# ferdean/lsa-fw

Hardware: AMD Instinct MI355X
Metric: converged eigenpairs/sec (k=20, shift-invert) (higher is better)
Workload: dtype c128

## Files before the change

lsa-fw_amd/csrc/dense.hip:

```cpp
#include <algorithm>
#include <chrono>
#include <cmath>
#include <cstdint>
#include <cstring>
#include <vector>

#include "lsa_internal.h"

namespace {

struct Z {
    double re, im;
};
inline Z operator+(Z a, Z b) { return {a.re + b.re, a.im + b.im}; }
inline Z operator-(Z a, Z b) { return {a.re - b.re, a.im - b.im}; }
inline Z operator-(Z a) { return {-a.re, -a.im}; }
inline Z operator*(Z a, Z b) { return {a.re * b.re - a.im * b.im, a.re * b.im + a.im * b.re}; }
inline Z operator*(double a, Z b) { return {a * b.re, a * b.im}; }
inline Z conj(Z a) { return {a.re, -a.im}; }
inline double abs1(Z a) { return std::fabs(a.re) + std::fabs(a.im); }
inline double abs2(Z a) { return a.re * a.re + a.im * a.im; }
inline double zabs(Z a) { return std::hypot(a.re, a.im); }
inline Z zdiv(Z a, Z b) {
    if (std::fabs(b.re) >= std::fabs(b.im)) {
// ... 921 lines not shown
    double* est_out;
    lsa_ks_result* result;
    int32_t m = 0;
    int64_t n = 0;
    int nev = 0, ldh = 0;
    double keep_fraction = 0.5;
    Selector sel;
    Rng rng;
    std::vector<Z> vec, H, T, Q, S, b, bq, w;
    std::vector<double> est, rel, keys;
    std::vector<int> rank;
    std::vector<char> select;
    int kept = 0, restarts = 0;
    int64_t applies = 0;
    KsClock clk;

    void random_vector() {
        for (int64_t i = 0; i < n; ++i) {
            rng.normal_pair(vec[(size_t)i].re, vec[(size_t)i].im);
            if (mask && mask[i] == 0.0) vec[(size_t)i] = {0.0, 0.0};
        }
    }
    int init(const char* who, const void* v0) {
        LSA_CHECK(lsa_krylov_shape(k, &n, &m));
        if (m > n) return lsa_set_error(ctx, LSA_ERR_ARG, "ncv = %d exceeds the problem size %lld", m, (long long)n);
        LSA_CHECK(ks_check_options(ctx, who, o, max_out, theta_out, lambda_out));
        nev = std::min<int>(o->nev, m);
        keep_fraction = ks_keep_fraction(o);
        sel = Selector{o->which, o->transform, {o->sigma[0], o->sigma[1]}, {o->antishift[0], o->antishift[1]}, {o->target[0], o->target[1]}};
        rng = ks_rng(o);
// ... 16 lines not shown
        select.resize((size_t)m);
        memset(result, 0, sizeof *result);
        return LSA_OK;
    }
    int extend(int j, int32_t* bd) {
        LSA_CHECK(lsa_krylov_extend(ctx, k, j, m, H.data(), ldh, bd));
        if (*bd >= 0) H[(size_t)*bd * ldh + (size_t)*bd + 1] = {0.0, 0.0};
        return (int)LSA_OK;
    }
    int inject_random(int j) {
        random_vector();
        return lsa_krylov_inject(ctx, k, j, vec.data());
    }
    int expand() {
        clk.start();
        LSA_CHECK(ks_expand(kept, m, &applies, [&](int j, int32_t* bd) { return extend(j, bd); }, [&](int j) { return inject_random(j); }));
        clk.lap(clk.expand);
        return LSA_OK;
    }
    int expand_after(int rc0, int32_t bd0, double seconds, int64_t* later_steps) {
        bool first = true;
        const int64_t before = applies + (bd0 < 0 ? m - kept : bd0 - kept + 1);
        *later_steps = 0;
        clk.start();
        LSA_CHECK(ks_expand(kept, m, &applies,
                            [&](int j, int32_t* bd) {
                                if (!first) return extend(j, bd);
                                first = false;
                                LSA_CHECK(rc0);
                                *bd = bd0;
// ... 2 lines not shown
                            },
                            [&](int j) { return inject_random(j); }));
        clk.lap(clk.expand);
        clk.expand += seconds;
        *later_steps = applies - before;
        return LSA_OK;
    }
    int after_expand(const char* who, bool* done) {
        const Mat Hm{H.data(), ldh}, Tm{T.data(), m}, Qm{Q.data(), m}, Sm{S.data(), m};
        *done = false;
        clk.start();
        for (int c = 0; c < m; ++c) {
            b[(size_t)c] = Hm(m, c);
            for (int r = 0; r < m; ++r) Tm(r, c) = Hm(r, c);
        }
        if (!schur(m, Tm, Qm)) return lsa_set_error(ctx, LSA_ERR_DIVERGED, "Krylov-Schur: the QR algorithm on the projected matrix did not converge");
        tri_eigenvectors(m, Tm, Sm);
        for (int c = 0; c < m; ++c) {
            Z acc = {0.0, 0.0};
            for (int r = 0; r < m; ++r) acc = acc + b[(size_t)r] * Qm(r, c);
            bq[(size_t)c] = acc;
        }
        for (int c = 0; c < m; ++c) {
            Z acc = {0.0, 0.0};
            for (int r = 0; r <= c; ++r) acc = acc + bq[(size_t)r] * Sm(r, c);
            est[(size_t)c] = zabs(acc);
            w[(size_t)c] = Tm(c, c);
            keys[(size_t)c] = sel.key(w[(size_t)c]);
            rel[(size_t)c] = est[(size_t)c] / std::max(zabs(w[(size_t)c]), 2.2250738585072014e-308);
        }
// ... 20 lines not shown
            clk.lap(clk.dense);
            ks_fill_result(result, clk, nconv, nout, restarts, applies, nconv < m ? rel[(size_t)rank[(size_t)nconv]] : 0.0);
            *done = true;
            return k_agree_in_step(ctx, who);
        }
        int knew = ks_keep_count(m, nconv, keep_fraction);
        {
            std::vector<double> sorted(keys);
            std::sort(sorted.begin(), sorted.end());
            const double thr = sorted[(size_t)knew] > sorted[(size_t)knew - 1] ? 0.5 * (sorted[(size_t)knew - 1] + sorted[(size_t)knew]) : sorted[(size_t)knew - 1];
            for (int c = 0; c < m; ++c) select[(size_t)c] = keys[(size_t)c] <= thr;
            const int sdim = schur_reorder(m, Tm, Qm, select);
            knew = std::max(std::min(sdim, m - 1), 1);
        }
        clk.lap(clk.dense);
        LSA_CHECK(lsa_krylov_restart(ctx, k, m, knew, Q.data(), m));
        clk.lap(clk.restart);
        std::fill(H.begin(), H.end(), Z{0.0, 0.0});
        for (int c = 0; c < knew; ++c) {
            for (int r = 0; r <= c; ++r) Hm(r, c) = Tm(r, c);
            Z acc = {0.0, 0.0};
            for (int r = 0; r < m; ++r) acc = acc + b[(size_t)r] * Qm(r, c);
            Hm(knew, c) = acc;
        }
        kept = knew;
        ++restarts;
        return LSA_OK;
    }
};

}

extern "C" {

int lsa_krylov_solve(lsa_ctx* ctx, lsa_krylov* k, const lsa_ks_options* o, const void* v0, const double* mask, int32_t max_out, void* theta_out,
                     void* lambda_out, void* X_out, double* est_out, lsa_ks_result* result) {
    if (!ctx || !k || !o || !result) return lsa_set_error(ctx, LSA_ERR_ARG, "lsa_krylov_solve: null argument");
    KsState st{ctx, k, o, mask, max_out, theta_out, lambda_out, X_out, est_out, result};
    LSA_CHECK(st.init("lsa_krylov_solve", v0));
    for (bool done = false; !done;) {
        LSA_CHECK(st.expand());
        LSA_CHECK(st.after_expand("lsa_krylov_solve", &done));
    }
    return LSA_OK;
}

static_assert(sizeof(lsa_ks_batch_info) == 288, "lsa_ks_batch_info layout is part of the C-ABI (tests/test_lockstep_cpu.py)");
static_assert(sizeof(((lsa_ks_batch_info*)nullptr)->lockstep_steps) == 8 * kKrylovGroupMax && sizeof(((lsa_ks_batch_info*)nullptr)->solo_steps) == 8 * kKrylovGroupMax,
              "the per-problem counters of lsa_ks_batch_info hold one entry per problem of a group");

int lsa_krylov_solve_batch(lsa_ctx* ctx, int32_t J, lsa_krylov* const* k, const lsa_ks_options* const* opts, const void* const* v0, int32_t max_out,
                           void* const* theta_out, void* const* lambda_out, void* const* X_out, double* const* est_out, lsa_ks_result* results,
                           int32_t* status, lsa_ks_batch_info* info) {
    if (!ctx || !k || !opts || !results || !status) return lsa_set_error(ctx, LSA_ERR_ARG, "lsa_krylov_solve_batch: null argument");
    if (J < 1 || J > kKrylovGroupMax) return lsa_set_error(ctx, LSA_ERR_ARG, "lsa_krylov_solve_batch: J = %d outside [1, %d]", J, kKrylovGroupMax);
    if (max_out > 0 && (!theta_out || !lambda_out)) return lsa_set_error(ctx, LSA_ERR_ARG, "lsa_krylov_solve_batch: output buffers are required");
    for (int32_t z = 0; z < J; ++z)
        if (!opts[z]) return lsa_set_error(ctx, LSA_ERR_ARG, "lsa_krylov_solve_batch: null options (problem %d)", z);
    LSA_CHECK(krylov_group_check(ctx, J, k));
// ... 152 lines not shown
```

lsa-fw_amd/csrc/lsa_internal.h:

```cpp
#pragma once

#include <hip/hip_runtime.h>

#include <cstdarg>
#include <cstdint>
#include <cstdio>
#include <cstdlib>
#include <cstring>
#include <memory>
#include <string>
#include <vector>

#include "../../include/lsa_hip.h"

struct cplx {
    double re, im;
};
static_assert(sizeof(cplx) == 16, "complex128 layout");

__host__ __device__ inline cplx make_cplx(double r, double i) { return cplx{r, i}; }

template <typename T>
struct scalar_traits;
template <>
// ... 214 lines not shown
int k_dcgs2_tail_batch(lsa_ctx* ctx, int J, int64_t n, const int32_t* j, void* const* V, int64_t ldv, const void* const* y, void* const* work,
                       const lsa_mat* const* M, const lsa_mat* const* C, void* const* t, double* const* tail_part, void* const* slot, int lds);
int k_spmv_plain_subwave_lanes(const lsa_mat* A);
int k_basis_gemm_max_cols(int dtype);
int k_basis_gemm(lsa_ctx* ctx, int dtype, int64_t n, int m, int k, const void* V, int64_t ldv, const void* Q, int ldq,
                 void* Out, int64_t ldo);
int k_scatter_rows(lsa_ctx* ctx, int dtype, int64_t n, int ncols, const int32_t* perm, const void* In, void* Out);

int basis_upload_row_permutation(lsa_ctx* ctx, const char* who, int64_t n, const int32_t* perm, int32_t** row_perm);
int basis_times_host_matrix(lsa_ctx* ctx, int dtype, int64_t n, int m, int k, const void* V, const void* Q, int ldq, void* qdev, void* Out,
                            size_t pinned_extra);
int direct_solve_enqueue(lsa_ctx* ctx, lsa_op* op, int dtype, const void* rhs, void* y, void* z, void* r, bool refine, double* norms,
                         int direction = -1);
void stats_book_direct_solve(lsa_stats* st, int products, bool refine, double res, double bnorm);

struct KrylovGroupBuf {
    int32_t J, slots, nparts;
    void* Hdev;
    double *checks, *tail_parts;
};
int krylov_group_check(lsa_ctx* ctx, int32_t J, lsa_krylov* const* ks);
int krylov_group_alloc(lsa_ctx* ctx, int32_t J, lsa_krylov* const* ks, KrylovGroupBuf* gb);
void krylov_group_free(KrylovGroupBuf* gb);
int krylov_extend_batch(lsa_ctx* ctx, KrylovGroupBuf* gb, lsa_krylov* const* ks, const uint8_t* active, const int32_t* j0, int32_t j1, void* const* Hs,
                        int32_t ldh, int32_t* breakdown, int32_t* status, std::string* errs, lsa_ks_batch_info* info);
void lsa_name_problem(lsa_ctx* ctx, int32_t z);

struct lsa_ndlu;
struct lsa_op_parts {
    int64_t n;
// ... 74 lines not shown
```

lsa-fw_amd/csrc/solver.hip:

```cpp
#include <algorithm>
#include <chrono>
#include <cmath>
#include <complex>

#include "lsa_internal.h"

int ilu_check_abort(lsa_ctx* ctx, lsa_ilu* pc);
bool nd_batch_compatible(const lsa_ndlu* f, const lsa_ndlu* g);
int ndlu_solve_batch_dev(lsa_ctx* ctx, int32_t J, lsa_ndlu* const* f, int vdtype, const void** b, void* const* x);
int k_allgather_inplace(lsa_ctx* ctx, void* vec, size_t bytes_per_rank);

namespace {

using zc = std::complex<double>;
inline size_t esize(int dtype) { return dtype == LSA_C128 ? 16 : 8; }
inline double now_s() {
    return std::chrono::duration<double>(std::chrono::steady_clock::now().time_since_epoch()).count();
}

struct KrylovSwitches {
    bool fused;
    bool four_passes;
    bool tail;
    bool delayed;
    bool timing;
};
const KrylovSwitches& krylov_switches() {
    static const KrylovSwitches sw = [] {
        const char* passes = getenv("LSA_KRYLOV_PASSES");
        return KrylovSwitches{env_flag("LSA_KRYLOV_FUSED", true), passes && atoi(passes) == 4, env_flag("LSA_KRYLOV_TAIL", true),
                              env_flag("LSA_KRYLOV_DELAYED", true), getenv("LSA_KRYLOV_TIMING") != nullptr};
    }();
    return sw;
}

struct OrthWork {
    void *h1 = nullptr, *h2 = nullptr, *hcol = nullptr;
    double* nrm2 = nullptr;
    void* fused = nullptr;
    int cap = 0;
    int ensure_fused(lsa_ctx* ctx, int64_t n) {
        if (fused) return LSA_OK;
        LSA_HIP_ALLOC(ctx, hipMalloc(&fused, k_cgs2_fused_work_bytes(ctx, n, cap)));
        return LSA_OK;
    }
    int alloc(lsa_ctx* ctx, int cap_, int dtype) {
// ... 404 lines not shown
    int32_t* row_perm = nullptr;
    void *V, *V2, *w, *qdev;
    OrthWork ow;
    std::vector<zc> hcol;
    double* imag2 = nullptr;
    void* xtmp = nullptr;
    std::vector<double> imag_norms;
    void* Hdev = nullptr;
    double* checks = nullptr;
    int32_t batch = 0;
    bool pipeline = false;
    void* w2 = nullptr;
    double* tail_parts = nullptr;
    int32_t tail_nparts = 0;
    int32_t t_for = -1;
};

static size_t krylov_slot_bytes(int32_t ncv) { return (size_t)(2 * ncv + 4) * 16; }

static void krylov_free(lsa_krylov* k) {
    for (void* p : {k->V, k->V2, k->w, k->qdev, k->Hdev, (void*)k->checks, (void*)k->imag2, k->xtmp, (void*)k->row_perm, k->w2, (void*)k->tail_parts})
        if (p) (void)hipFree(p);
    k->ow.release();
    delete k;
}

extern "C" {

int lsa_gmres(lsa_ctx* ctx, const lsa_mat* C, lsa_ilu* pc, const lsa_vec* b, lsa_vec* x, int use_x0, double rtol, int restart,
              int maxit, int32_t* iters, double* rel_res) {
    if (!ctx || !C || !b || !x) return lsa_set_error(ctx, LSA_ERR_ARG, "lsa_gmres: null argument");
    if (C->n != C->ncols || b->n != C->n || x->n != C->n || b->dtype != x->dtype)
        return lsa_set_error(ctx, LSA_ERR_ARG, "lsa_gmres: shape/dtype mismatch");
    if (C->dtype == LSA_C128 && b->dtype != LSA_C128) return lsa_set_error(ctx, LSA_ERR_ARG, "lsa_gmres: complex matrix needs complex vectors");
    if (restart < 1 || maxit < 1 || !(rtol > 0.0)) return lsa_set_error(ctx, LSA_ERR_ARG, "lsa_gmres: restart, maxit, rtol must be positive");
    restart = std::min(restart, maxit);
    if (restart > k_basis_gemm_max_cols(b->dtype))
// ... 367 lines not shown
    return LSA_OK;
}

int lsa_krylov_create(lsa_ctx* ctx, lsa_op* op, int32_t ncv, lsa_krylov** out) {
    if (!ctx || !op || !out || ncv < 1) return lsa_set_error(ctx, LSA_ERR_ARG, "lsa_krylov_create: bad argument");
    if (ncv > k_basis_gemm_max_cols(LSA_C128))
        return lsa_set_error(ctx, LSA_ERR_ARG, "lsa_krylov_create: ncv=%d, the basis product handles at most %d basis vectors", ncv, k_basis_gemm_max_cols(LSA_C128));
    const size_t vb = (size_t)std::max<int64_t>(op->n, 1) * 16;
    const char* be = getenv("LSA_KRYLOV_BATCH");
    const int32_t batch = be && *be ? std::max(0, std::min(atoi(be), 256)) : 16;
    if (lsa_krylov* c = ctx->krylov_cache) {
        ctx->krylov_cache = nullptr;
        if (c->n == op->n && c->ncv == ncv && c->batch == batch) {
            c->op = op;
            c->pipeline = true;
            c->imag_norms.clear();
            (void)hipMemsetAsync(c->w, 0, vb, ctx->stream);
            *out = c;
            return LSA_OK;
        }
        krylov_free(c);
    }
    lsa_krylov* k = new lsa_krylov();
    k->ctx = ctx;
    k->op = op;
    k->n = op->n;
    k->ncv = ncv;
    k->V = k->V2 = k->w = k->qdev = nullptr;
    bool ok = hipMalloc(&k->V, vb * (size_t)(ncv + 1)) == hipSuccess && hipMalloc(&k->V2, vb * (size_t)(ncv + 1)) == hipSuccess &&
              hipMalloc(&k->w, vb) == hipSuccess && hipMalloc(&k->qdev, (size_t)(ncv + 1) * (size_t)(ncv + 1) * 16) == hipSuccess;
    if (!ok || k->ow.alloc(ctx, ncv + 1, LSA_C128) != LSA_OK) {
        lsa_krylov_destroy(k);
        return lsa_set_error(ctx, LSA_ERR_HIP, "lsa_krylov_create: out of device memory (n=%lld, ncv=%d)", (long long)op->n, ncv);
    }
    (void)hipMemsetAsync(k->w, 0, vb, ctx->stream);
    k->hcol.assign((size_t)ncv + 2, zc(0));
    k->batch = batch;
    const size_t slots = (size_t)std::max(batch, 1);
    if (hipMalloc(&k->Hdev, slots * krylov_slot_bytes(ncv)) != hipSuccess || hipMalloc((void**)&k->checks, slots * 2 * sizeof(double)) != hipSuccess) {
        lsa_krylov_destroy(k);
        return lsa_set_error(ctx, LSA_ERR_HIP, "lsa_krylov_create: out of device memory (pipeline buffers)");
    }
    k->pipeline = true;
    *out = k;
    return LSA_OK;
}

void lsa_krylov_destroy(lsa_krylov* k) {
    if (!k) return;
    lsa_ctx* ctx = k->ctx;
    if (ctx && ctx->stream) (void)hipStreamSynchronize(ctx->stream);
    if (k->row_perm) (void)hipFree(k->row_perm);
    k->row_perm = nullptr;
// ... 15 lines not shown

int lsa_krylov_shape(const lsa_krylov* k, int64_t* n, int32_t* ncv) {
    if (!k) return LSA_ERR_ARG;
    if (n) *n = k->n;
    if (ncv) *ncv = k->ncv;
    return LSA_OK;
}

int lsa_krylov_set_row_permutation(lsa_ctx* ctx, lsa_krylov* k, const int32_t* perm) {
    if (!ctx || !k) return lsa_set_error(ctx, LSA_ERR_ARG, "lsa_krylov_set_row_permutation: null argument");
    return basis_upload_row_permutation(ctx, "lsa_krylov_set_row_permutation", k->n, perm, &k->row_perm);
}

int lsa_krylov_set_start(lsa_ctx* ctx, lsa_krylov* k, const void* host_v) {
    if (!ctx || !k || !host_v) return lsa_set_error(ctx, LSA_ERR_ARG, "lsa_krylov_set_start: null argument");
    LSA_HIP_CHECK(ctx, hipMemcpyAsync(k->w, host_v, (size_t)k->n * 16, hipMemcpyHostToDevice, ctx->stream));
    double nrm = 0.0;
    LSA_CHECK(device_norm(ctx, LSA_C128, k->n, k->w, k->ow.nrm2, &nrm));
    if (!(nrm > 0.0) || !std::isfinite(nrm)) return lsa_set_error(ctx, LSA_ERR_ARG, "lsa_krylov_set_start: start vector is zero or not finite");
    LSA_CHECK(k_scale_by_inv_norm(ctx, LSA_C128, k->n, k->w, k->ow.nrm2, k->V));
    LSA_HIP_CHECK(ctx, hipStreamSynchronize(ctx->stream));
    k->pipeline = true;
    return LSA_OK;
}

int lsa_krylov_inject(lsa_ctx* ctx, lsa_krylov* k, int32_t j, const void* host_v) {
    if (!ctx || !k || !host_v) return lsa_set_error(ctx, LSA_ERR_ARG, "lsa_krylov_inject: null argument");
    if (j < 0 || j > k->ncv) return lsa_set_error(ctx, LSA_ERR_ARG, "lsa_krylov_inject: index %d out of range", j);
    if (j == 0) return lsa_krylov_set_start(ctx, k, host_v);
    const size_t vb = (size_t)k->n * 16;
    LSA_HIP_CHECK(ctx, hipMemcpyAsync(k->w, host_v, vb, hipMemcpyHostToDevice, ctx->stream));
    LSA_CHECK(orthonormalize(ctx, LSA_C128, k->n, k->V, k->n, j, k->w, (char*)k->V + (size_t)j * vb, k->ow, k->hcol.data()));
    const double beta = k->hcol[j].real();
    if (!(beta > 0.0) || !std::isfinite(beta)) return lsa_set_error(ctx, LSA_ERR_ARG, "lsa_krylov_inject: vector lies in the span of the basis");
    return LSA_OK;
}

enum class Orth {
    cgs2_fused,
    cgs2_staged,
    dcgs2,
};
struct StepPlan {
    bool pipelined = false;
// ... 12 lines not shown
    p.tail = p.pipelined && sw.tail && sw.fused && op->Kmul && !op->adjoint && !op->keep && !op->refine && op->n == k->n &&
             k_cgs2_tail_fits(ctx, k->n, k->ncv, op->Kmul, op->Kfac);
    return p;
}

static int krylov_enqueue_step(lsa_ctx* ctx, lsa_krylov* k, const StepPlan& plan, int32_t j, int32_t slot, bool first) {
    lsa_op* op = k->op;
    const int dtype = LSA_C128;
    const size_t vb = (size_t)k->n * 16;
    const void* vj = (char*)k->V + (size_t)j * vb;
    void* vn = (char*)k->V + (size_t)(j + 1) * vb;
    void* sl = (char*)k->Hdev + (size_t)slot * krylov_slot_bytes(k->ncv);
    double* chk = k->checks + 2 * (size_t)slot;
    const bool dcgs2 = plan.orth == Orth::dcgs2;
    if (plan.orth != Orth::cgs2_staged) LSA_CHECK(k->ow.ensure_fused(ctx, k->n));
    if (plan.tail) {
        if (k->t_for != j) LSA_CHECK(spmv_global(ctx, op->Kmul, dtype, vj, op->t, false));
        k->t_for = -1;
        LSA_CHECK(pc_global(ctx, pc_of(op), op->Kfac->row0, op->n, dtype, op->t, k->w));
        double* parts = k->tail_parts + (size_t)slot * 2 * (size_t)k->tail_nparts;
        if (dcgs2) {
            LSA_CHECK(k_dcgs2_step(ctx, k->n, j, k->V, k->n, k->w, first ? 1 : 0, sl, k->ncv, k->ow.fused, nullptr, nullptr, nullptr));
            LSA_CHECK(k_dcgs2_tail(ctx, k->n, j, k->V, k->n, k->w, k->ow.fused, op->Kmul, op->Kfac, op->t, parts, sl, k->ncv));
        } else {
            LSA_CHECK(k_cgs2_fused_tail(ctx, k->n, j + 1, k->V, k->n, k->w, k->w2, vn, sl, k->ow.fused, op->Kmul, op->Kfac, op->t, parts));
        }
        k->t_for = j + 1;
        return LSA_OK;
    }
    k->t_for = -1;
    const void* rhs = vj;
    if (op->Kmul) {
        LSA_CHECK(spmv_global(ctx, op->Kmul, dtype, vj, op->t, op->adjoint));
        rhs = op->t;
// ... 60 lines not shown

static int arnoldi_nonfinite(lsa_ctx* ctx, int32_t j) { return lsa_set_error(ctx, LSA_ERR_NONFINITE, "Arnoldi: non-finite norm at step %d", j); }

struct ExtendCursor {
    int32_t j;
    bool pending;
};

static int pipelined_prepare(lsa_ctx* ctx, lsa_krylov* k, const StepPlan& plan) {
    lsa_op* op = k->op;
    if (!op->gw_ready) {
        LSA_CHECK(op->gw.alloc(ctx, op->n, std::max(1, std::min({op->opts.ksp_restart, op->opts.ksp_maxit, 40})), LSA_C128));
        op->gw_ready = true;
    }
    if (plan.tail && !k->tail_parts) {
        const int32_t slots = std::max(k->batch, 1);
        k->tail_nparts = k_cgs2_tail_parts(k->n);
        LSA_HIP_ALLOC(ctx, hipMalloc(&k->w2, (size_t)k->n * 16));
        LSA_HIP_ALLOC(ctx, hipMalloc((void**)&k->tail_parts, (size_t)slots * 2 * (size_t)k->tail_nparts * sizeof(double)));
    }
    return LSA_OK;
}

static int accept_steps(lsa_ctx* ctx, lsa_krylov* k, const HessView& H, bool delayed, const char* slots, size_t slot_stride, const double* chk,
                        size_t chk_stride, int32_t nb, ExtendCursor* c, int32_t* breakdown, int32_t* accepted_out) {
    lsa_op* op = k->op;
    const double rtol = op->opts.ksp_rtol;
    cplx* hwork = (cplx*)k->hcol.data();
    const int32_t j = c->j;
    int32_t accepted = 0;
    *accepted_out = 0;
    for (int32_t s = 0; s < nb; ++s, ++accepted) {
        const cplx* hc = (const cplx*)(slots + (size_t)s * slot_stride);
        const bool first = s == 0 && !c->pending;
        if (delayed && !first) {
// ... 19 lines not shown
            *breakdown = j + s;
            return LSA_OK;
        }
    }
    c->j = j + accepted;
    *accepted_out = accepted;
    if (accepted < nb) k->t_for = -1;
    return LSA_OK;
}

static int extend_pipelined(lsa_ctx* ctx, lsa_krylov* k, const HessView& H, ExtendCursor* c, int32_t j1, int32_t* breakdown) {
    StepPlan plan = step_plan(ctx, k);
    LSA_CHECK(pipelined_prepare(ctx, k, plan));
    const int32_t slots = std::max(k->batch, 1);
    const size_t colb = krylov_slot_bytes(k->ncv);
    LSA_CHECK(lsa_ensure_scratch(ctx, 0, (size_t)slots * (colb + 2 * sizeof(double))));
    const bool delayed = plan.orth == Orth::dcgs2;
    char* host = (char*)ctx->pinned;
    k->t_for = -1;
    for (; c->j < j1 && plan.pipelined; plan = step_plan(ctx, k)) {
        const int32_t nb = std::min<int32_t>(slots, j1 - c->j);
        const double tq = now_s();
        for (int32_t s = 0; s < nb; ++s) {
            const int rc = krylov_enqueue_step(ctx, k, plan, c->j + s, s, s == 0 && !c->pending);
            if (rc != LSA_OK) {
                (void)hipStreamSynchronize(ctx->stream);
                return rc;
            }
        }
        if (plan.tail) LSA_CHECK(k_cgs2_tail_checks(ctx, nb, k->tail_nparts, k->tail_parts, k->checks));
        LSA_HIP_CHECK(ctx, hipMemcpyAsync(host, k->Hdev, (size_t)nb * colb, hipMemcpyDeviceToHost, ctx->stream));
        LSA_HIP_CHECK(ctx, hipMemcpyAsync(host + (size_t)slots * colb, k->checks, (size_t)nb * 2 * sizeof(double), hipMemcpyDeviceToHost, ctx->stream));
        const double tw = now_s();
        LSA_HIP_CHECK(ctx, hipStreamSynchronize(ctx->stream));
        if (krylov_switches().timing) fprintf(stderr, "[lsa_krylov] %d steps queued in %.3f ms, waited %.3f ms\n", nb, 1e3 * (tw - tq), 1e3 * (now_s() - tw));
        int32_t accepted = 0;
        LSA_CHECK(accept_steps(ctx, k, H, delayed, host, colb, (const double*)(host + (size_t)slots * colb), 2, nb, c, breakdown, &accepted));
        if (*breakdown >= 0) return LSA_OK;
    }
    if (c->pending) {
        const int32_t j = c->j;
        LSA_CHECK(k_dcgs2_step(ctx, k->n, j, k->V, k->n, nullptr, 0, k->Hdev, k->ncv, k->ow.fused, nullptr, nullptr, nullptr));
        LSA_HIP_CHECK(ctx, hipMemcpyAsync(host, k->Hdev, colb, hipMemcpyDeviceToHost, ctx->stream));
        LSA_HIP_CHECK(ctx, hipStreamSynchronize(ctx->stream));
        c->pending = false;
        const int what = finish_column(H, j, (const cplx*)host);
        if (what < 0) return arnoldi_nonfinite(ctx, j - 1);
        if (what > 0) *breakdown = j - 1;
    }
    return LSA_OK;
}

static int extend_one_step(lsa_ctx* ctx, lsa_krylov* k, const HessView& H, int32_t j, int32_t j1, int32_t* breakdown) {
    const size_t vb = (size_t)k->n * 16;
    k->t_for = -1;
    for (; j < j1; ++j) {
        const void* vj = (char*)k->V + (size_t)j * vb;
        void* vn = (char*)k->V + (size_t)(j + 1) * vb;
        LSA_CHECK(op_apply_dev(ctx, k->op, vj, k->w));
        LSA_CHECK(orthonormalize(ctx, LSA_C128, k->n, k->V, k->n, j + 1, k->w, vn, k->ow, k->hcol.data()));
        const int what = take_column(H, j, (const cplx*)k->hcol.data());
        if (what < 0) return arnoldi_nonfinite(ctx, j);
        if (what > 0) {
            *breakdown = j;
            break;
        }
    }
    return LSA_OK;
}

static int extend_rest(lsa_ctx* ctx, lsa_krylov* k, const HessView& H, ExtendCursor* c, int32_t j1, int32_t* bd) {
    int rc = LSA_OK;
    if (step_plan(ctx, k).pipelined) rc = extend_pipelined(ctx, k, H, c, j1, bd);
    if (rc == LSA_OK && *bd < 0) rc = extend_one_step(ctx, k, H, c->j, j1, bd);
    return rc;
}

int lsa_krylov_extend(lsa_ctx* ctx, lsa_krylov* k, int32_t j0, int32_t j1, void* H, int32_t ldh, int32_t* breakdown) {
    if (!ctx || !k || !H) return lsa_set_error(ctx, LSA_ERR_ARG, "lsa_krylov_extend: null argument");
    if (j0 < 0 || j1 < j0 || j1 > k->ncv || ldh < j1 + 1) return lsa_set_error(ctx, LSA_ERR_ARG, "lsa_krylov_extend: bad step range [%d, %d) for ncv %d", j0, j1, k->ncv);
    const double t0 = now_s();
    const HessView Hv{(cplx*)H, ldh, j0, k->ncv};
    ExtendCursor c{j0, false};
    int32_t bd = -1;
    const int rc = extend_rest(ctx, k, Hv, &c, j1, &bd);
    if (breakdown) *breakdown = bd;
    k->op->st.seconds_solve += now_s() - t0;
    return rc;
}

}

int krylov_group_alloc(lsa_ctx* ctx, int32_t J, lsa_krylov* const* ks, KrylovGroupBuf* gb) {
    memset(gb, 0, sizeof *gb);
    gb->J = J;
    gb->slots = std::max(ks[0]->batch, 1);
    gb->nparts = k_cgs2_tail_parts(ks[0]->n);
    const size_t cells = (size_t)J * (size_t)gb->slots;
    LSA_HIP_ALLOC(ctx, hipMalloc(&gb->Hdev, cells * krylov_slot_bytes(ks[0]->ncv)));
    LSA_HIP_ALLOC(ctx, hipMalloc((void**)&gb->checks, cells * 2 * sizeof(double)));
    LSA_HIP_ALLOC(ctx, hipMalloc((void**)&gb->tail_parts, cells * 2 * (size_t)gb->nparts * sizeof(double)));
    LSA_HIP_CHECK(ctx, hipMemsetAsync(gb->tail_parts, 0, cells * 2 * (size_t)gb->nparts * sizeof(double), ctx->stream));
    return LSA_OK;
}

// ... 31 lines not shown
        HessView H;
        bool lock;
        int32_t nb;
    } mem[kKrylovGroupMax];
    int32_t nactive = 0;
    int32_t ncv = 0;
    for (int32_t z = 0; z < J; ++z) {
        mem[z] = Member{ExtendCursor{0, false}, HessView{nullptr, 0, 0, 0}, false, 0};
        if (!active[z]) continue;
        ++nactive;
        ncv = ks[z]->ncv;
        breakdown[z] = -1;
        status[z] = LSA_OK;
        mem[z] = Member{ExtendCursor{j0[z], false}, HessView{(cplx*)Hs[z], ldh, j0[z], ks[z]->ncv}, true, 0};
        ks[z]->t_for = -1;
    }
    const size_t colb = krylov_slot_bytes(ncv);
    const size_t cells = (size_t)J * (size_t)slots;
    while (true) {
        int32_t lead = -1, rounds = 0;
        for (int32_t z = 0; z < J; ++z) {
            Member& m = mem[z];
            m.nb = 0;
            if (!active[z] || !m.lock || status[z] != LSA_OK || breakdown[z] >= 0 || m.c.j >= j1) continue;
            lsa_krylov* k = ks[z];
            const StepPlan plan = step_plan(ctx, k);
            bool in = plan.pipelined && plan.orth == Orth::dcgs2 && plan.tail;
            if (in && lead >= 0)
                in = nd_batch_compatible(ks[lead]->op->nd, k->op->nd) && ks[lead]->op->Kmul->dtype == k->op->Kmul->dtype;
            if (!in) {
// ... 92 lines not shown
        const int xrc = extend_rest(ctx, ks[z], mem[z].H, &mem[z].c, j1, &breakdown[z]);
        if (xrc != LSA_OK) fail(z, xrc);
        else if (info) info->solo_steps[z] += (breakdown[z] >= 0 ? breakdown[z] + 1 : j1) - jb;
    }
    const double share = (now_s() - t0) / std::max(nactive, 1);
    for (int32_t z = 0; z < J; ++z)
        if (active[z]) ks[z]->op->st.seconds_solve += share;
    return LSA_OK;
}

extern "C" {

int lsa_krylov_restart(lsa_ctx* ctx, lsa_krylov* k, int32_t m, int32_t knew, const void* Q, int32_t ldq) {
    if (!ctx || !k || !Q) return lsa_set_error(ctx, LSA_ERR_ARG, "lsa_krylov_restart: null argument");
    if (m < 1 || m > k->ncv || knew < 0 || knew > m || ldq < m) return lsa_set_error(ctx, LSA_ERR_ARG, "lsa_krylov_restart: bad sizes m=%d knew=%d", m, knew);
    const size_t vb = (size_t)k->n * 16;
    if (knew > 0) LSA_CHECK(basis_times_host_matrix(ctx, LSA_C128, k->n, m, knew, k->V, Q, ldq, k->qdev, k->V2, 0));
    LSA_CHECK(k_copy(ctx, LSA_C128, k->n, (char*)k->V + (size_t)m * vb, (char*)k->V2 + (size_t)knew * vb));
    LSA_HIP_CHECK(ctx, hipStreamSynchronize(ctx->stream));
    std::swap(k->V, k->V2);
    return LSA_OK;
}

int lsa_krylov_ritz_vectors(lsa_ctx* ctx, lsa_krylov* k, int32_t m, int32_t nvec, const void* Y, int32_t ldy, int normalise,
                            void* X) {
    if (!ctx || !k || !Y || !X) return lsa_set_error(ctx, LSA_ERR_ARG, "lsa_krylov_ritz_vectors: null argument");
    if (m < 1 || m > k->ncv + 1 || nvec < 0 || nvec > k->ncv + 1 || ldy < m) return lsa_set_error(ctx, LSA_ERR_ARG, "lsa_krylov_ritz_vectors: bad sizes");
    if (nvec == 0) return LSA_OK;
    const size_t vb = (size_t)k->n * 16;
    LSA_CHECK(basis_times_host_matrix(ctx, LSA_C128, k->n, m, nvec, k->V, Y, ldy, k->qdev, k->V2, (size_t)nvec * sizeof(double)));
    k->imag_norms.clear();
    if (normalise & 2) {
        if (!k->imag2) LSA_HIP_ALLOC(ctx, hipMalloc((void**)&k->imag2, (size_t)(k->ncv + 2) * sizeof(double)));
        LSA_CHECK(k_columns_canonical(ctx, k->n, nvec, k->V2, k->n, normalise & 1, k->imag2));
        k->imag_norms.assign((size_t)nvec, 0.0);
        LSA_HIP_CHECK(ctx, hipMemcpyAsync((char*)ctx->pinned + (size_t)m * nvec * 16, k->imag2, (size_t)nvec * sizeof(double), hipMemcpyDeviceToHost, ctx->stream));
    } else if (normalise) {
        for (int32_t c = 0; c < nvec; ++c) {
            void* col = (char*)k->V2 + (size_t)c * vb;
            LSA_CHECK(k_nrm2(ctx, LSA_C128, k->n, col, k->ow.nrm2));
            LSA_CHECK(k_copy(ctx, LSA_C128, k->n, col, k->w));
            LSA_CHECK(k_scale_by_inv_norm(ctx, LSA_C128, k->n, k->w, k->ow.nrm2, col));
        }
    }
    const void* src = k->V2;
    void* tmp = nullptr;
    if (k->row_perm) {
        if (!k->xtmp) LSA_HIP_ALLOC(ctx, hipMalloc(&k->xtmp, vb * (size_t)(k->ncv + 1)));
        tmp = k->xtmp;
        LSA_CHECK(k_scatter_rows(ctx, LSA_C128, k->n, nvec, k->row_perm, k->V2, tmp));
        src = tmp;
    }
    hipError_t e = hipMemcpyAsync(X, src, vb * (size_t)nvec, hipMemcpyDeviceToHost, ctx->stream);
    if (e == hipSuccess) e = hipStreamSynchronize(ctx->stream);
    if (e != hipSuccess) return lsa_set_error(ctx, LSA_ERR_HIP, "lsa_krylov_ritz_vectors: download failed: %s", hipGetErrorString(e));
    for (size_t c = 0; c < k->imag_norms.size(); ++c) k->imag_norms[c] = std::sqrt(((const double*)((const char*)ctx->pinned + (size_t)m * nvec * 16))[c]);
    return LSA_OK;
}

int lsa_krylov_imag_norms(const lsa_krylov* k, int32_t nvec, double* out) {
    if (!k || !out || nvec < 0 || (size_t)nvec > k->imag_norms.size()) return LSA_ERR_ARG;
    for (int32_t c = 0; c < nvec; ++c) out[c] = k->imag_norms[(size_t)c];
    return LSA_OK;
}

int lsa_eig_residuals(lsa_ctx* ctx, const lsa_mat* A, const lsa_mat* M, int32_t nvec, const void* lam, const void* X, double* res) {
    if (!ctx || !A || !lam || !X || !res || nvec < 0) return lsa_set_error(ctx, LSA_ERR_ARG, "lsa_eig_residuals: bad argument");
    const int64_t n = A->n;
    const size_t vb = (size_t)std::max<int64_t>(n, 1) * 16;
    void *x = nullptr, *ax = nullptr, *mx = nullptr;
// ... 70 lines not shown
```

Measured before the change: 585.6.

## Double-buffer Arnoldi batches and pre-apply shift-invert operator during host dense work

Arnoldi step batches now run on two sets of device slots and pinned host regions with per-set events, so the next batch is queued on the stream before the host accepts the current one. In the single-solve path, the operator (SpMV plus preconditioner solve) for column m is queued before the host runs the Schur decomposition, and the restart no longer synchronises the stream, so device work overlaps host dense linear algebra. This adds speculative work that is discarded on breakdown, partial acceptance or injection, plus more bookkeeping state that must stay consistent.

```diff
diff --git a/lsa-fw_amd/csrc/dense.hip b/lsa-fw_amd/csrc/dense.hip
--- a/lsa-fw_amd/csrc/dense.hip
+++ b/lsa-fw_amd/csrc/dense.hip
@@ -959,6 +959,7 @@
     int kept = 0, restarts = 0;
     int64_t applies = 0;
     KsClock clk;
+    bool ahead = false;
 
     void random_vector() {
         for (int64_t i = 0; i < n; ++i) {
@@ -1005,6 +1006,7 @@
     }
     int expand() {
         clk.start();
+        krylov_arm_preapply(k, ahead && restarts < o->max_restarts);
         LSA_CHECK(ks_expand(kept, m, &applies, [&](int j, int32_t* bd) { return extend(j, bd); }, [&](int j) { return inject_random(j); }));
         clk.lap(clk.expand);
         return LSA_OK;
@@ -1037,6 +1039,7 @@
             b[(size_t)c] = Hm(m, c);
             for (int r = 0; r < m; ++r) Tm(r, c) = Hm(r, c);
         }
+        if (ahead && restarts < o->max_restarts) LSA_CHECK(krylov_preapply(ctx, k, m));
         if (!schur(m, Tm, Qm)) return lsa_set_error(ctx, LSA_ERR_DIVERGED, "Krylov-Schur: the QR algorithm on the projected matrix did not converge");
         tri_eigenvectors(m, Tm, Sm);
         for (int c = 0; c < m; ++c) {
@@ -1087,7 +1090,7 @@
             knew = std::max(std::min(sdim, m - 1), 1);
         }
         clk.lap(clk.dense);
-        LSA_CHECK(lsa_krylov_restart(ctx, k, m, knew, Q.data(), m));
+        LSA_CHECK(ahead ? krylov_restart_queued(ctx, k, m, knew, Q.data(), m) : lsa_krylov_restart(ctx, k, m, knew, Q.data(), m));
         clk.lap(clk.restart);
         std::fill(H.begin(), H.end(), Z{0.0, 0.0});
         for (int c = 0; c < knew; ++c) {
@@ -1111,11 +1114,14 @@
     if (!ctx || !k || !o || !result) return lsa_set_error(ctx, LSA_ERR_ARG, "lsa_krylov_solve: null argument");
     KsState st{ctx, k, o, mask, max_out, theta_out, lambda_out, X_out, est_out, result};
     LSA_CHECK(st.init("lsa_krylov_solve", v0));
-    for (bool done = false; !done;) {
-        LSA_CHECK(st.expand());
-        LSA_CHECK(st.after_expand("lsa_krylov_solve", &done));
-    }
-    return LSA_OK;
+    st.ahead = true;
+    int rc = LSA_OK;
+    for (bool done = false; !done && rc == LSA_OK;) {
+        rc = st.expand();
+        if (rc == LSA_OK) rc = st.after_expand("lsa_krylov_solve", &done);
+    }
+    krylov_arm_preapply(k, false);
+    return rc;
 }
 
 static_assert(sizeof(lsa_ks_batch_info) == 288, "lsa_ks_batch_info layout is part of the C-ABI (tests/test_lockstep_cpu.py)");
diff --git a/lsa-fw_amd/csrc/lsa_internal.h b/lsa-fw_amd/csrc/lsa_internal.h
--- a/lsa-fw_amd/csrc/lsa_internal.h
+++ b/lsa-fw_amd/csrc/lsa_internal.h
@@ -252,6 +252,10 @@
                          int direction = -1);
 void stats_book_direct_solve(lsa_stats* st, int products, bool refine, double res, double bnorm);
 
+void krylov_arm_preapply(lsa_krylov* k, bool on);
+int krylov_preapply(lsa_ctx* ctx, lsa_krylov* k, int32_t m);
+int krylov_restart_queued(lsa_ctx* ctx, lsa_krylov* k, int32_t m, int32_t knew, const void* Q, int32_t ldq);
+
 struct KrylovGroupBuf {
     int32_t J, slots, nparts;
     void* Hdev;
diff --git a/lsa-fw_amd/csrc/solver.hip b/lsa-fw_amd/csrc/solver.hip
--- a/lsa-fw_amd/csrc/solver.hip
+++ b/lsa-fw_amd/csrc/solver.hip
@@ -24,12 +24,13 @@
     bool tail;
     bool delayed;
     bool timing;
+    bool preapply;
 };
 const KrylovSwitches& krylov_switches() {
     static const KrylovSwitches sw = [] {
         const char* passes = getenv("LSA_KRYLOV_PASSES");
         return KrylovSwitches{env_flag("LSA_KRYLOV_FUSED", true), passes && atoi(passes) == 4, env_flag("LSA_KRYLOV_TAIL", true),
-                              env_flag("LSA_KRYLOV_DELAYED", true), getenv("LSA_KRYLOV_TIMING") != nullptr};
+                              env_flag("LSA_KRYLOV_DELAYED", true), getenv("LSA_KRYLOV_TIMING") != nullptr, env_flag("LSA_KRYLOV_PREAPPLY", true)};
     }();
     return sw;
 }
@@ -464,6 +465,16 @@
     double* tail_parts = nullptr;
     int32_t tail_nparts = 0;
     int32_t t_for = -1;
+    bool pre_armed = false;
+    int32_t pre_col = -1, pre_for = -1;
+    const lsa_op* pre_op = nullptr;
+    void drop_preapply() { pre_col = pre_for = -1; }
+    hipEvent_t ev_read[2] = {nullptr, nullptr};
+    int ensure_events(lsa_ctx* ctx_) {
+        for (hipEvent_t& e : ev_read)
+            if (!e) LSA_HIP_CHECK(ctx_, hipEventCreateWithFlags(&e, hipEventDisableTiming));
+        return LSA_OK;
+    }
 };
 
 static size_t krylov_slot_bytes(int32_t ncv) { return (size_t)(2 * ncv + 4) * 16; }
@@ -471,6 +482,8 @@
 static void krylov_free(lsa_krylov* k) {
     for (void* p : {k->V, k->V2, k->w, k->qdev, k->Hdev, (void*)k->checks, (void*)k->imag2, k->xtmp, (void*)k->row_perm, k->w2, (void*)k->tail_parts})
         if (p) (void)hipFree(p);
+    for (hipEvent_t e : k->ev_read)
+        if (e) (void)hipEventDestroy(e);
     k->ow.release();
     delete k;
 }
@@ -868,6 +881,8 @@
         if (c->n == op->n && c->ncv == ncv && c->batch == batch) {
             c->op = op;
             c->pipeline = true;
+            c->pre_armed = false;
+            c->drop_preapply();
             c->imag_norms.clear();
             (void)hipMemsetAsync(c->w, 0, vb, ctx->stream);
             *out = c;
@@ -890,7 +905,7 @@
     (void)hipMemsetAsync(k->w, 0, vb, ctx->stream);
     k->hcol.assign((size_t)ncv + 2, zc(0));
     k->batch = batch;
-    const size_t slots = (size_t)std::max(batch, 1);
+    const size_t slots = 2 * (size_t)std::max(batch, 1);
     if (hipMalloc(&k->Hdev, slots * krylov_slot_bytes(ncv)) != hipSuccess || hipMalloc((void**)&k->checks, slots * 2 * sizeof(double)) != hipSuccess) {
         lsa_krylov_destroy(k);
         return lsa_set_error(ctx, LSA_ERR_HIP, "lsa_krylov_create: out of device memory (pipeline buffers)");
@@ -936,6 +951,8 @@
 
 int lsa_krylov_set_start(lsa_ctx* ctx, lsa_krylov* k, const void* host_v) {
     if (!ctx || !k || !host_v) return lsa_set_error(ctx, LSA_ERR_ARG, "lsa_krylov_set_start: null argument");
+    k->pre_armed = false;
+    k->drop_preapply();
     LSA_HIP_CHECK(ctx, hipMemcpyAsync(k->w, host_v, (size_t)k->n * 16, hipMemcpyHostToDevice, ctx->stream));
     double nrm = 0.0;
     LSA_CHECK(device_norm(ctx, LSA_C128, k->n, k->w, k->ow.nrm2, &nrm));
@@ -950,6 +967,7 @@
     if (!ctx || !k || !host_v) return lsa_set_error(ctx, LSA_ERR_ARG, "lsa_krylov_inject: null argument");
     if (j < 0 || j > k->ncv) return lsa_set_error(ctx, LSA_ERR_ARG, "lsa_krylov_inject: index %d out of range", j);
     if (j == 0) return lsa_krylov_set_start(ctx, k, host_v);
+    k->drop_preapply();
     const size_t vb = (size_t)k->n * 16;
     LSA_HIP_CHECK(ctx, hipMemcpyAsync(k->w, host_v, vb, hipMemcpyHostToDevice, ctx->stream));
     LSA_CHECK(orthonormalize(ctx, LSA_C128, k->n, k->V, k->n, j, k->w, (char*)k->V + (size_t)j * vb, k->ow, k->hcol.data()));
@@ -992,10 +1010,12 @@
     double* chk = k->checks + 2 * (size_t)slot;
     const bool dcgs2 = plan.orth == Orth::dcgs2;
     if (plan.orth != Orth::cgs2_staged) LSA_CHECK(k->ow.ensure_fused(ctx, k->n));
+    const bool ahead = plan.tail && dcgs2 && first && k->pre_for == j && k->pre_op == op;
+    k->drop_preapply();
     if (plan.tail) {
-        if (k->t_for != j) LSA_CHECK(spmv_global(ctx, op->Kmul, dtype, vj, op->t, false));
+        if (!ahead && k->t_for != j) LSA_CHECK(spmv_global(ctx, op->Kmul, dtype, vj, op->t, false));
         k->t_for = -1;
-        LSA_CHECK(pc_global(ctx, pc_of(op), op->Kfac->row0, op->n, dtype, op->t, k->w));
+        if (!ahead) LSA_CHECK(pc_global(ctx, pc_of(op), op->Kfac->row0, op->n, dtype, op->t, k->w));
         double* parts = k->tail_parts + (size_t)slot * 2 * (size_t)k->tail_nparts;
         if (dcgs2) {
             LSA_CHECK(k_dcgs2_step(ctx, k->n, j, k->V, k->n, k->w, first ? 1 : 0, sl, k->ncv, k->ow.fused, nullptr, nullptr, nullptr));
@@ -1086,11 +1106,27 @@
         op->gw_ready = true;
     }
     if (plan.tail && !k->tail_parts) {
-        const int32_t slots = std::max(k->batch, 1);
+        const int32_t slots = 2 * std::max(k->batch, 1);
         k->tail_nparts = k_cgs2_tail_parts(k->n);
         LSA_HIP_ALLOC(ctx, hipMalloc(&k->w2, (size_t)k->n * 16));
         LSA_HIP_ALLOC(ctx, hipMalloc((void**)&k->tail_parts, (size_t)slots * 2 * (size_t)k->tail_nparts * sizeof(double)));
     }
+    return LSA_OK;
+}
+
+static int preapply_enqueue(lsa_ctx* ctx, lsa_krylov* k, int32_t m) {
+    if (k->pre_col == m && k->pre_op == k->op) return LSA_OK;
+    k->drop_preapply();
+    if (!krylov_switches().preapply || m < 1 || m > k->ncv) return LSA_OK;
+    const StepPlan plan = step_plan(ctx, k);
+    if (!(plan.pipelined && plan.tail && plan.orth == Orth::dcgs2)) return LSA_OK;
+    LSA_CHECK(pipelined_prepare(ctx, k, plan));
+    lsa_op* op = k->op;
+    k->t_for = -1;
+    LSA_CHECK(spmv_global(ctx, op->Kmul, LSA_C128, (char*)k->V + (size_t)m * (size_t)k->n * 16, op->t, false));
+    LSA_CHECK(pc_global(ctx, pc_of(op), op->Kfac->row0, op->n, LSA_C128, op->t, k->w));
+    k->pre_col = m;
+    k->pre_op = op;
     return LSA_OK;
 }
 
@@ -1140,37 +1176,103 @@
     LSA_CHECK(pipelined_prepare(ctx, k, plan));
     const int32_t slots = std::max(k->batch, 1);
     const size_t colb = krylov_slot_bytes(k->ncv);
-    LSA_CHECK(lsa_ensure_scratch(ctx, 0, (size_t)slots * (colb + 2 * sizeof(double))));
+    const size_t region = (size_t)slots * (colb + 2 * sizeof(double));
+    LSA_CHECK(lsa_ensure_scratch(ctx, 0, 2 * region));
     const bool delayed = plan.orth == Orth::dcgs2;
-    char* host = (char*)ctx->pinned;
+    const bool ahead = krylov_switches().preapply;
+    if (ahead) LSA_CHECK(k->ensure_events(ctx));
     k->t_for = -1;
-    for (; c->j < j1 && plan.pipelined; plan = step_plan(ctx, k)) {
-        const int32_t nb = std::min<int32_t>(slots, j1 - c->j);
+    struct Queued {
+        int32_t j, nb, set;
+    };
+    auto host_of = [&](int32_t set) { return (char*)ctx->pinned + (size_t)set * region; };
+    auto slot_of = [&](int32_t set) { return (char*)k->Hdev + (size_t)set * (size_t)slots * colb; };
+    auto queued = [&](int32_t set) -> int {
+        if (ahead) LSA_HIP_CHECK(ctx, hipEventRecord(k->ev_read[set], ctx->stream));
+        return LSA_OK;
+    };
+    auto wait_for = [&](const Queued& q) -> int {
+        const double tw = now_s();
+        if (ahead) LSA_HIP_CHECK(ctx, hipEventSynchronize(k->ev_read[q.set]));
+        else LSA_HIP_CHECK(ctx, hipStreamSynchronize(ctx->stream));
+        if (krylov_switches().timing) fprintf(stderr, "[lsa_krylov] %d steps from %d: waited %.3f ms\n", q.nb, q.j, 1e3 * (now_s() - tw));
+        return LSA_OK;
+    };
+    auto queue_batch = [&](const StepPlan& p, int32_t j, bool first, int32_t set, Queued* q) -> int {
+        const int32_t nb = std::min<int32_t>(slots, j1 - j);
         const double tq = now_s();
         for (int32_t s = 0; s < nb; ++s) {
-            const int rc = krylov_enqueue_step(ctx, k, plan, c->j + s, s, s == 0 && !c->pending);
+            const int rc = krylov_enqueue_step(ctx, k, p, j + s, set * slots + s, s == 0 && first);
             if (rc != LSA_OK) {
                 (void)hipStreamSynchronize(ctx->stream);
                 return rc;
             }
         }
-        if (plan.tail) LSA_CHECK(k_cgs2_tail_checks(ctx, nb, k->tail_nparts, k->tail_parts, k->checks));
-        LSA_HIP_CHECK(ctx, hipMemcpyAsync(host, k->Hdev, (size_t)nb * colb, hipMemcpyDeviceToHost, ctx->stream));
-        LSA_HIP_CHECK(ctx, hipMemcpyAsync(host + (size_t)slots * colb, k->checks, (size_t)nb * 2 * sizeof(double), hipMemcpyDeviceToHost, ctx->stream));
-        const double tw = now_s();
+        double* chk = k->checks + 2 * (size_t)set * (size_t)slots;
+        if (p.tail) LSA_CHECK(k_cgs2_tail_checks(ctx, nb, k->tail_nparts, k->tail_parts + (size_t)set * (size_t)slots * 2 * (size_t)k->tail_nparts, chk));
+        LSA_HIP_CHECK(ctx, hipMemcpyAsync(host_of(set), slot_of(set), (size_t)nb * colb, hipMemcpyDeviceToHost, ctx->stream));
+        LSA_HIP_CHECK(ctx, hipMemcpyAsync(host_of(set) + (size_t)slots * colb, chk, (size_t)nb * 2 * sizeof(double), hipMemcpyDeviceToHost, ctx->stream));
+        LSA_CHECK(queued(set));
+        if (krylov_switches().timing) fprintf(stderr, "[lsa_krylov] %d steps from %d queued in %.3f ms\n", nb, j, 1e3 * (now_s() - tq));
+        *q = Queued{j, nb, set};
+        return LSA_OK;
+    };
+    auto queue_flush = [&](int32_t j, int32_t set, Queued* q) -> int {
+        LSA_CHECK(k_dcgs2_step(ctx, k->n, j, k->V, k->n, nullptr, 0, slot_of(set), k->ncv, k->ow.fused, nullptr, nullptr, nullptr));
+        LSA_HIP_CHECK(ctx, hipMemcpyAsync(host_of(set), slot_of(set), colb, hipMemcpyDeviceToHost, ctx->stream));
+        LSA_CHECK(queued(set));
+        if (k->pre_armed && j == k->ncv) LSA_CHECK(preapply_enqueue(ctx, k, j));
+        *q = Queued{j, 0, set};
+        return LSA_OK;
+    };
+    auto drain = [&]() -> int {
+        k->t_for = -1;
+        k->drop_preapply();
         LSA_HIP_CHECK(ctx, hipStreamSynchronize(ctx->stream));
-        if (krylov_switches().timing) fprintf(stderr, "[lsa_krylov] %d steps queued in %.3f ms, waited %.3f ms\n", nb, 1e3 * (tw - tq), 1e3 * (now_s() - tw));
+        return LSA_OK;
+    };
+    Queued cur{0, 0, 0}, next{0, 0, 0};
+    bool have = false, flushed = false;
+    if (c->j < j1 && plan.pipelined) {
+        LSA_CHECK(queue_batch(plan, c->j, !c->pending, 0, &cur));
+        have = true;
+    }
+    while (have) {
+        bool have_next = false;
+        if (ahead) {
+            const int32_t jn = cur.j + cur.nb;
+            if (jn < j1) LSA_CHECK(queue_batch(plan, jn, !delayed, cur.set ^ 1, &next));
+            else if (delayed) LSA_CHECK(queue_flush(jn, cur.set ^ 1, &next));
+            have_next = jn < j1 || delayed;
+        }
+        LSA_CHECK(wait_for(cur));
         int32_t accepted = 0;
-        LSA_CHECK(accept_steps(ctx, k, H, delayed, host, colb, (const double*)(host + (size_t)slots * colb), 2, nb, c, breakdown, &accepted));
-        if (*breakdown >= 0) return LSA_OK;
+        const char* host = host_of(cur.set);
+        const int arc = accept_steps(ctx, k, H, delayed, host, colb, (const double*)(host + (size_t)slots * colb), 2, cur.nb, c, breakdown, &accepted);
+        if (arc != LSA_OK || *breakdown >= 0) {
+            if (have_next) (void)drain();
+            return arc;
+        }
+        if (accepted == cur.nb && have_next) {
+            cur = next;
+            if (cur.nb == 0) {
+                flushed = true;
+                break;
+            }
+            continue;
+        }
+        if (have_next) LSA_CHECK(drain());
+        plan = step_plan(ctx, k);
+        have = c->j < j1 && plan.pipelined;
+        if (have) LSA_CHECK(queue_batch(plan, c->j, !c->pending, 0, &cur));
     }
     if (c->pending) {
         const int32_t j = c->j;
-        LSA_CHECK(k_dcgs2_step(ctx, k->n, j, k->V, k->n, nullptr, 0, k->Hdev, k->ncv, k->ow.fused, nullptr, nullptr, nullptr));
-        LSA_HIP_CHECK(ctx, hipMemcpyAsync(host, k->Hdev, colb, hipMemcpyDeviceToHost, ctx->stream));
-        LSA_HIP_CHECK(ctx, hipStreamSynchronize(ctx->stream));
+        if (!flushed) LSA_CHECK(queue_flush(j, 0, &cur));
+        LSA_CHECK(wait_for(cur));
         c->pending = false;
-        const int what = finish_column(H, j, (const cplx*)host);
+        const int what = finish_column(H, j, (const cplx*)host_of(cur.set));
+        if (what != 0) k->drop_preapply();
         if (what < 0) return arnoldi_nonfinite(ctx, j - 1);
         if (what > 0) *breakdown = j - 1;
     }
@@ -1180,6 +1282,7 @@
 static int extend_one_step(lsa_ctx* ctx, lsa_krylov* k, const HessView& H, int32_t j, int32_t j1, int32_t* breakdown) {
     const size_t vb = (size_t)k->n * 16;
     k->t_for = -1;
+    if (j < j1) k->drop_preapply();
     for (; j < j1; ++j) {
         const void* vj = (char*)k->V + (size_t)j * vb;
         void* vn = (char*)k->V + (size_t)(j + 1) * vb;
@@ -1209,12 +1312,34 @@
     const HessView Hv{(cplx*)H, ldh, j0, k->ncv};
     ExtendCursor c{j0, false};
     int32_t bd = -1;
+    if (k->pre_for != j0 || j0 >= j1) k->drop_preapply();
     const int rc = extend_rest(ctx, k, Hv, &c, j1, &bd);
+    k->pre_for = -1;
     if (breakdown) *breakdown = bd;
     k->op->st.seconds_solve += now_s() - t0;
     return rc;
 }
 
+}
+
+void krylov_arm_preapply(lsa_krylov* k, bool on) { k->pre_armed = on && krylov_switches().preapply; }
+
+int krylov_preapply(lsa_ctx* ctx, lsa_krylov* k, int32_t m) { return k->pre_armed ? preapply_enqueue(ctx, k, m) : (int)LSA_OK; }
+
+static int krylov_restart_impl(lsa_ctx* ctx, lsa_krylov* k, int32_t m, int32_t knew, const void* Q, int32_t ldq, bool queued) {
+    const size_t vb = (size_t)k->n * 16;
+    const int32_t ahead = k->pre_col == m && k->pre_op == k->op ? knew : -1;
+    k->drop_preapply();
+    if (knew > 0) LSA_CHECK(basis_times_host_matrix(ctx, LSA_C128, k->n, m, knew, k->V, Q, ldq, k->qdev, k->V2, 0));
+    LSA_CHECK(k_copy(ctx, LSA_C128, k->n, (char*)k->V + (size_t)m * vb, (char*)k->V2 + (size_t)knew * vb));
+    if (!queued) LSA_HIP_CHECK(ctx, hipStreamSynchronize(ctx->stream));
+    std::swap(k->V, k->V2);
+    k->pre_for = ahead;
+    return LSA_OK;
+}
+
+int krylov_restart_queued(lsa_ctx* ctx, lsa_krylov* k, int32_t m, int32_t knew, const void* Q, int32_t ldq) {
+    return krylov_restart_impl(ctx, k, m, knew, Q, ldq, krylov_switches().preapply && step_plan(ctx, k).pipelined);
 }
 
 int krylov_group_alloc(lsa_ctx* ctx, int32_t J, lsa_krylov* const* ks, KrylovGroupBuf* gb) {
@@ -1276,6 +1401,7 @@
         status[z] = LSA_OK;
         mem[z] = Member{ExtendCursor{j0[z], false}, HessView{(cplx*)Hs[z], ldh, j0[z], ks[z]->ncv}, true, 0};
         ks[z]->t_for = -1;
+        ks[z]->drop_preapply();
     }
     const size_t colb = krylov_slot_bytes(ncv);
     const size_t cells = (size_t)J * (size_t)slots;
@@ -1398,12 +1524,7 @@
 int lsa_krylov_restart(lsa_ctx* ctx, lsa_krylov* k, int32_t m, int32_t knew, const void* Q, int32_t ldq) {
     if (!ctx || !k || !Q) return lsa_set_error(ctx, LSA_ERR_ARG, "lsa_krylov_restart: null argument");
     if (m < 1 || m > k->ncv || knew < 0 || knew > m || ldq < m) return lsa_set_error(ctx, LSA_ERR_ARG, "lsa_krylov_restart: bad sizes m=%d knew=%d", m, knew);
-    const size_t vb = (size_t)k->n * 16;
-    if (knew > 0) LSA_CHECK(basis_times_host_matrix(ctx, LSA_C128, k->n, m, knew, k->V, Q, ldq, k->qdev, k->V2, 0));
-    LSA_CHECK(k_copy(ctx, LSA_C128, k->n, (char*)k->V + (size_t)m * vb, (char*)k->V2 + (size_t)knew * vb));
-    LSA_HIP_CHECK(ctx, hipStreamSynchronize(ctx->stream));
-    std::swap(k->V, k->V2);
-    return LSA_OK;
+    return krylov_restart_impl(ctx, k, m, knew, Q, ldq, false);
 }
 
 int lsa_krylov_ritz_vectors(lsa_ctx* ctx, lsa_krylov* k, int32_t m, int32_t nvec, const void* Y, int32_t ldy, int normalise,
@@ -1412,6 +1533,7 @@
     if (m < 1 || m > k->ncv + 1 || nvec < 0 || nvec > k->ncv + 1 || ldy < m) return lsa_set_error(ctx, LSA_ERR_ARG, "lsa_krylov_ritz_vectors: bad sizes");
     if (nvec == 0) return LSA_OK;
     const size_t vb = (size_t)k->n * 16;
+    k->drop_preapply();
     LSA_CHECK(basis_times_host_matrix(ctx, LSA_C128, k->n, m, nvec, k->V, Y, ldy, k->qdev, k->V2, (size_t)nvec * sizeof(double)));
     k->imag_norms.clear();
     if (normalise & 2) {
@@ -1435,9 +1557,13 @@
         LSA_CHECK(k_scatter_rows(ctx, LSA_C128, k->n, nvec, k->row_perm, k->V2, tmp));
         src = tmp;
     }
+    const bool timing = krylov_switches().timing;
+    if (timing) LSA_HIP_CHECK(ctx, hipStreamSynchronize(ctx->stream));
+    const double td = now_s();
     hipError_t e = hipMemcpyAsync(X, src, vb * (size_t)nvec, hipMemcpyDeviceToHost, ctx->stream);
     if (e == hipSuccess) e = hipStreamSynchronize(ctx->stream);
     if (e != hipSuccess) return lsa_set_error(ctx, LSA_ERR_HIP, "lsa_krylov_ritz_vectors: download failed: %s", hipGetErrorString(e));
+    if (timing) fprintf(stderr, "[lsa_krylov] %d Ritz vectors of %lld rows downloaded in %.3f ms\n", nvec, (long long)k->n, 1e3 * (now_s() - td));
     for (size_t c = 0; c < k->imag_norms.size(); ++c) k->imag_norms[c] = std::sqrt(((const double*)((const char*)ctx->pinned + (size_t)m * nvec * 16))[c]);
     return LSA_OK;
 }
```

Result: faster. 603.7 (median of 6 runs) (+3.1%).
